# chongkuiqi/S2ANet

Hardware: AMD Instinct MI355X
Metric: 1024x1024 DOTA chips/sec (R-50-FPN S2ANet inference) (higher is better)
Workload: dtype f16; 1 GPU; BASELINE configs[2]: full R-50-FPN S2ANet inference, batch 8 of 1024x1024 synthetic uint8 chips per GPU; 3 independent batches in flight on 3 HIP streams; global_batch=8, num_classes=15, weights=seeded random init of the reference architecture; odm_cls bias calibrated, nms_candidate_cap=160000, nms_candidates_dropped=0, distinct_input_batches=3, fam_cls_branch=True, hip_graph=False, batches_in_flight=3, parallelism=dp1 (one process per GPU)

## Files before the change

### include/s2anet_hip.h

```cpp
#ifndef S2ANET_HIP_H_
#define S2ANET_HIP_H_

#include <stddef.h>
#include <stdint.h>

#ifdef __cplusplus
extern "C" {
#endif

#define S2A_OK 0
#define S2A_EINVAL (-1)
#define S2A_EWORKSPACE (-2)
#define S2A_EHIP (-3)
#define S2A_ENOTIMPL (-4)

#define S2A_DTYPE_F32 0
#define S2A_DTYPE_F16 1
#define S2A_DTYPE_F64 2

#define S2A_LAYOUT_NCHW 0
#define S2A_LAYOUT_NHWC 1

typedef void* s2a_stream_t;

// ... 258 lines not shown
int s2a_deform_conv_backward_typed(int dtype, const void* input, const void* offset, const void* grad_output,
                                   const void* weight, void* grad_input, void* grad_offset, float* grad_weight_f32,
                                   float scale, int64_t batch, int64_t channels, int64_t height, int64_t width,
                                   int64_t out_channels, void* workspace, size_t workspace_bytes, s2a_stream_t stream);

int s2a_conv3x3_tail1x1_f16(const void* x, const void* weight_frag, const void* bias, const void* tail_weight_frag,
                            const void* tail_bias, const void* residual, void* out, const void* chain_weight_frag,
                            const void* chain_bias, void* chain_out, int64_t chain_channels, int64_t batch, int64_t channels,
                            int64_t mid_channels, int64_t out_channels, int64_t height, int64_t width,
                            s2a_stream_t stream);

int s2a_conv1x1_chain_f16(const void* x, const void* weight_frag, const void* bias, const void* residual, void* out,
                          const void* chain_weight_frag, const void* chain_bias, void* chain_out, int64_t chain_channels,
                          int64_t batch, int64_t channels, int64_t out_channels, int64_t height, int64_t width,
                          s2a_stream_t stream);

int s2a_conv1x1_add_up2_f16(const void* x, const void* weight_frag, const void* bias, const void* coarse,
                            void* out, int64_t batch, int64_t channels, int64_t height, int64_t width,
                            int64_t out_channels, s2a_stream_t stream);
int s2a_sum_pool2x2_f16(const void* g, void* out, int64_t batch, int64_t height, int64_t width, int64_t channels,
                        s2a_stream_t stream);

int64_t s2a_pyramid_pixels(const s2a_pyramid* pyr, int64_t batch);
int s2a_conv3x3_pyramid_f16(const void* x, const void* weight_frag, const void* bias, const void* residual,
                            void* out, int64_t batch, int64_t channels, int64_t out_channels, int relu,
                            const s2a_pyramid* pyr, s2a_stream_t stream);
int s2a_conv3x3_head_pyramid_f16(const void* x, const void* weight_frag, const void* bias, void* out,
                                 const void* head_weight_frag, const void* head_bias, void* head_out,
                                 int64_t batch, int64_t channels, int64_t out_channels, int relu,
                                 const s2a_pyramid* pyr, s2a_stream_t stream);
// ... 125 lines not shown
```

### s2anet_amd/_lib.py

```python
import ctypes
import os
import subprocess

import torch

_HERE = os.path.dirname(os.path.abspath(__file__))
LIB_PATH = os.environ.get("S2A_LIB_PATH") or os.path.join(_HERE, "libs2anet_hip.so")

OK, EINVAL, EWORKSPACE, EHIP, ENOTIMPL = 0, -1, -2, -3, -4
DTYPE_F32, DTYPE_F16, DTYPE_F64 = 0, 1, 2
LAYOUT_NCHW, LAYOUT_NHWC = 0, 1

c_i64, c_int, c_f32, c_sz, c_vp = (ctypes.c_int64, ctypes.c_int, ctypes.c_float, ctypes.c_size_t,
                                   ctypes.c_void_p)


class DcnParams(ctypes.Structure):
    _fields_ = [("batch", c_i64), ("channels", c_i64), ("height", c_i64), ("width", c_i64),
                ("out_channels", c_i64),
                ("kW", c_int), ("kH", c_int), ("dW", c_int), ("dH", c_int), ("padW", c_int),
                ("padH", c_int), ("dilationW", c_int), ("dilationH", c_int), ("group", c_int),
                ("deformable_group", c_int), ("dtype", c_int), ("offset_dtype", c_int),
                ("layout", c_int), ("relu", c_int)]

# ... 137 lines not shown
                                               c_i64, c_vp, c_sz, c_vp]),
    "s2a_deform_conv_backward_input_f32_workspace_bytes": (c_sz, [c_i64, c_i64, c_i64, c_i64, c_i64]),
    "s2a_deform_conv_backward_weight_f32_workspace_bytes": (c_sz, [c_i64, c_i64, c_i64, c_i64, c_i64]),
    "s2a_deform_conv_backward_weight_f32": (c_int, [c_vp, c_vp, c_vp, c_vp, c_f32, c_i64, c_i64, c_i64, c_i64, c_i64,
                                                    c_vp, c_sz, c_vp]),
    "s2a_deform_conv_backward_input_f32": (c_int, [c_vp, c_vp, c_vp, c_vp, c_vp, c_vp, c_i64, c_i64, c_i64, c_i64, c_i64,
                                                   c_vp, c_sz, c_vp]),
    "s2a_deform_conv_backward_weight_f16": (c_int, [c_vp, c_vp, c_vp, c_vp, c_i64, c_i64, c_i64, c_i64, c_i64, c_vp, c_sz, c_vp]),
    "s2a_deform_conv_backward_input_f16": (c_int, [c_vp, c_vp, c_vp, c_vp, c_vp, c_vp, c_i64, c_i64, c_i64, c_i64, c_i64,
                                           c_vp, c_sz, c_vp]),
    "s2a_deformable_im2col": (c_int, [c_vp, c_vp, c_vp, ctypes.POINTER(DcnParams), c_vp]),
    "s2a_deformable_col2im": (c_int, [c_vp, c_vp, c_vp, ctypes.POINTER(DcnParams), c_vp]),
    "s2a_deformable_col2im_coord": (c_int, [c_vp, c_vp, c_vp, c_vp, ctypes.POINTER(DcnParams), c_vp]),
    "s2a_conv3x3_tail1x1_f16": (c_int, [c_vp] * 10 + [c_i64] * 7 + [c_vp]),
    "s2a_conv1x1_chain_f16": (c_int, [c_vp] * 8 + [c_i64] * 6 + [c_vp]),
    "s2a_conv1x1_add_up2_f16": (c_int, [c_vp, c_vp, c_vp, c_vp, c_vp, c_i64, c_i64, c_i64, c_i64, c_i64, c_vp]),
    "s2a_sum_pool2x2_f16": (c_int, [c_vp, c_vp, c_i64, c_i64, c_i64, c_i64, c_vp]),
    "s2a_pyramid_pixels": (c_i64, [ctypes.POINTER(Pyramid), c_i64]),
    "s2a_conv3x3_pyramid_f16": (c_int, [c_vp, c_vp, c_vp, c_vp, c_vp, c_i64, c_i64, c_i64, c_int,
                                        ctypes.POINTER(Pyramid), c_vp]),
    "s2a_conv3x3_head_pyramid_f16": (c_int, [c_vp, c_vp, c_vp, c_vp, c_vp, c_vp, c_vp, c_i64, c_i64, c_i64, c_int,
                                             ctypes.POINTER(Pyramid), c_vp]),
    "s2a_conv3x3_narrow_pyramid_f16": (c_int, [c_vp, c_vp, c_vp, c_vp, c_i64, c_i64, c_i64, c_int, ctypes.POINTER(Pyramid), c_vp]),
    "s2a_orconv_pool_pyramid_f16": (c_int, [c_vp, c_vp, c_vp, c_vp, c_vp, c_i64, c_i64, c_i64, ctypes.POINTER(Pyramid), c_vp]),
    "s2a_conv_wino_packed_elems": (c_i64, [c_i64, c_i64]),
    "s2a_conv_wino_pack_weight_f16": (c_int, [c_vp, c_i64, c_i64, c_vp, c_vp]),
    "s2a_conv3x3_wino_pyramid_f16": (c_int, [c_vp, c_vp, c_vp, c_vp, c_vp, c_i64, c_i64, c_i64, c_int,
                                             ctypes.POINTER(Pyramid), c_vp]),
    "s2a_quantize_e4m3": (c_int, [c_vp, c_vp, c_i64, c_i64, c_f32, c_vp]),
    "s2a_conv_pack_weight_fp8": (c_int, [c_vp, c_i64, c_i64, c_vp, c_vp]),
# ... 130 lines not shown
```

### s2anet_amd/csrc/conv_ops.hip

```cpp
#include <hip/hip_fp16.h>
#include <hip/hip_runtime.h>

#include <algorithm>
#include <cstdlib>
#include <type_traits>

#include "common.hpp"
#include "mfma_common.hpp"

namespace s2a {
namespace {

__global__ void k_pack_weight_frag(const _Float16* __restrict__ w, int O, int C, _Float16* __restrict__ wp,
                                   int taps = 9) {
  int64_t e = (int64_t)blockIdx.x * blockDim.x + threadIdx.x;
  int64_t total = (int64_t)O * C * taps;
  if (e >= total) return;
  const int G = O / 64;
  int j = (int)(e & 7);
  int lane = (int)((e >> 3) & 63);
  int kk = (int)((e >> 9) & 3);
  int mt = (int)((e >> 11) & 1);
  int64_t r = e >> 12;
  int g = (int)(r % G);
// ... 10 lines not shown
  _Float16* pool_out;
  const _Float16* head_w;
  const _Float16* head_b;
  _Float16* head_out;
  int store_main;
  const _Float16* tail_w;
  const _Float16* tail_b;
  const _Float16* tail_res;
  _Float16* tail_out;
  const _Float16* chain_w;
  const _Float16* chain_b;
  _Float16* chain_out;
  int chain_O;
};

template <int TAPS, int OG, int PH = 1, int SD = 1, bool TAIL = false, int HT = 0>
struct ConvCfg {
  static constexpr int kTH = (SD == 2 || HT) ? 4 : 8 * PH;
  static constexpr int kPos = (SD == 2 || HT) ? 64 : 128 * PH;
  static constexpr int kWaves = 4 * PH;
  static constexpr int kPW = SD == 2 ? 33 : kCPW;
  static constexpr int kNT = (kPos / 32) * OG / 4 / PH;
  static constexpr int kPix = TAPS == 9 ? ((kTH - 1) * SD + 3) * kPW : kPos;
  static constexpr int kDma = (kPix * 9 + 63) / 64;
  static constexpr int kPatchBytes = kDma * 1024;
  static constexpr int kOutRowB = OG * 128 + 16;
  static constexpr bool kWLds = PH == 2 && TAPS == 9;
  static constexpr int kWBuf = OG * 8192;
  static constexpr int kLoop0 = 2 * kPatchBytes + (kWLds ? 2 * kWBuf : 0);
  static constexpr int kLoop = (kWLds && OG == 1 && kPatchBytes + 9 * 8192 > kLoop0) ? kPatchBytes + 9 * 8192 : kLoop0;
  static constexpr int kLds0 = (kLoop > kPos * kOutRowB) ? kLoop : kPos * kOutRowB;
  static constexpr int kTailRowB = 528;
  static constexpr int kLds = (TAIL && kPos * kTailRowB > kLds0) ? kPos * kTailRowB : kLds0;
  static constexpr int kBiasBytes = TAIL ? 1024 : 512;
  static constexpr int kJ = (kDma + kWaves - 1) / kWaves;
};

template <int TAPS, int OG, int PH = 1, int SD = 1, bool TAIL = false, int HT = 0>
__global__ __launch_bounds__(256 * PH, PH == 1 ? 2 : 1) void k_conv_f16(const _Float16* __restrict__ x_,
                                                     const _Float16* __restrict__ wfrag,
                                                     const _Float16* __restrict__ bias,
                                                     const _Float16* __restrict__ residual_,
                                                     _Float16* __restrict__ out_, int64_t Ntot_, int C,
                                                     int H_, int W_, int Ho_, int Wo_, int cstride, int O,
                                                     int relu, unsigned x_bytes_, LevelTab lt, int res_up,
                                                     ConvExtra ex) {
  _Float16* pool_out_ = ex.pool_out;
  using T = _Float16;
  using V = f16x8;
  using Cfg = ConvCfg<TAPS, OG, PH, SD, TAIL, HT>;
  constexpr int NT = Cfg::kNT;
  static_assert(NT >= 1, "unsupported tile / group combination");
  static_assert(!HT || (TAPS == 9 && PH == 1 && SD == 1 && !TAIL), "half tiles: plain 3x3 / stride 1");
  static_assert(!TAIL || (TAPS == 9 && OG == 1 && SD == 1), "the fused 1x1 tail follows a 64-map 3x3/s1");
  constexpr int WPG = 4 / OG;
  constexpr int kThreads_ = 256 * PH;
  extern __shared__ __attribute__((aligned(16))) char smem[];
  const int tid = threadIdx.x, lane = tid & 63, wave = tid >> 6;
  const int wave4 = wave & 3, blk = wave >> 2;
  int64_t tile = xcd_remap(blockIdx.x, gridDim.x);
  const T* x = x_;
  const T* residual = residual_;
  T* out = out_;
  int64_t Ntot = Ntot_;
  int H = H_, W = W_, Ho = Ho_, Wo = Wo_;
  unsigned x_bytes = x_bytes_;
  if (TAPS == 9 && lt.n > 1) {
// ... 45 lines not shown
    }
    pvoff[j] = in ? (unsigned)(pix * row_bytes + q * 16) : 0x80000000u;
  }
  T* s_bias = reinterpret_cast<T*>(smem + Cfg::kLds);
  T bias_v = (T)0.f;
  if (bias && tid < Oloc) bias_v = bias[o0 + tid];
  T tail_bias_v = (T)0.f;
  V wt[2][4];
  if constexpr (TAIL) {
    if (tid < 256) tail_bias_v = ex.tail_b[tid];
    const V* tp = reinterpret_cast<const V*>(ex.tail_w) + (int64_t)wave4 * 8 * 64 + ((lane >> 4) & 1) * 128 + (lane >> 5) * 32 + (lane & 15);
#pragma unroll
    for (int f = 0; f < 8; f++) wt[f >> 2][f & 3] = tp[((f >> 2) * 4 + (f & 1)) * 64 + ((f >> 1) & 1) * 16];
  }
  auto patch_issue = [&](int cc) {
    char* P = smem + (cc & 1) * Cfg::kPatchBytes;
#pragma unroll
    for (int j = 0; j < Cfg::kJ; j++) {
      const int i = wave_u + Cfg::kWaves * j;
      if (i < Cfg::kDma)
        __builtin_amdgcn_raw_ptr_buffer_load_lds(rx, (__attribute__((address_space(3))) void*)(P + i * 1024), 16,
                                                 (int)pvoff[j], cc * 128, 0, 0);
    }
  };

  const int grp = wave4 / WPG, sub = wave4 % WPG;
  const bool wave_active = grp * 64 < Oloc;
  const int g = min(o0 / 64 + grp, G - 1);
  const V* wf_base = reinterpret_cast<const V*>(wfrag) + lane;
  V wA[2][4], wB[2][4];
  constexpr bool M16 = (TAPS == 9 && SD == 1) || (TAPS == 1 && OG == 4);
// ... 166 lines not shown
        if (t == 0 && cc + 1 < CC) patch_issue(cc + 1);
        compute_wl(Pc, t, wb + (s & 1) * Cfg::kWBuf);
        __syncthreads();
      }
    }
    }
  } else {
  patch_issue(0);
  load_w(0, wA);
  if (tid < 64 * OG) s_bias[tid] = bias_v;
  if constexpr (TAIL) { if (tid < 256) s_bias[64 + tid] = tail_bias_v; }
  __syncthreads();
  if constexpr (TAPS == 9) {
    for (int cc = 0; cc < CC; cc++) {
      const int s0 = cc * 9;
      const char* Pc = smem + (cc & 1) * Cfg::kPatchBytes;
#define S2A_TAP(T_, WCUR, WNEXT)                                                     \
      load_w(min(s0 + (T_) + 1, last), WNEXT);                                          \
      compute(Pc, (T_), WCUR);                                                          \
      __builtin_amdgcn_sched_barrier(0);
      S2A_TAP(0, wA, wB)
      S2A_TAP(1, wB, wA)
      S2A_TAP(2, wA, wB)
      S2A_TAP(3, wB, wA)
      S2A_TAP(4, wA, wB)
      S2A_TAP(5, wB, wA)
      if (cc + 1 < CC) patch_issue(cc + 1);
      S2A_TAP(6, wA, wB)
      S2A_TAP(7, wB, wA)
      S2A_TAP(8, wA, wB)
#undef S2A_TAP
      __syncthreads();
#pragma unroll
      for (int a = 0; a < 2; a++)
#pragma unroll
        for (int kk = 0; kk < 4; kk++) wA[a][kk] = wB[a][kk];
    }
  } else {
#define S2A_STAGE(C_, WCUR, WNEXT)                                                   \
    if ((C_) + 1 < CC) patch_issue((C_) + 1);                                           \
    load_w(min((C_) + 1, last), WNEXT);                                                 \
    compute(smem + ((C_) & 1) * Cfg::kPatchBytes, 0, WCUR);                             \
    __syncthreads();
    int cc = 0;
    for (; cc + 1 < CC; cc += 2) {
      S2A_STAGE(cc, wA, wB)
      S2A_STAGE(cc + 1, wB, wA)
// ... 666 lines not shown
    }
    stage_sync(issued);
#pragma unroll
    for (int i = 0; i < 4; i++) {
      const int idx = tid + 256 * i, pos = idx >> 3, col = idx & 7;
      const int y = cur.ty0 + (pos >> 4), xq = cur.tx0 + (pos & 15);
      V v;
#pragma unroll
      for (int e = 0; e < 8; e++) v[e] = (_Float16)0.f;
      if (col < 2) v = *reinterpret_cast<const V*>(so + pos * 32 + col * 16);
      if (y < cur.H && xq < cur.W) *reinterpret_cast<V*>(out + (cur.base + (int64_t)y * cur.W + xq) * 64 + col * 8) = v;
    }
  }
}

}
}

using namespace s2a;

namespace s2a {
namespace {
template <int TAPS, int OG, int PH = 1, int SD = 1, bool TAIL = false, int HT = 0>
int launch_conv(const _Float16* x, const _Float16* wfrag, const _Float16* bias, const _Float16* residual,
                _Float16* out, int64_t B, int C, int H, int W, int Ho, int Wo, int cstride, int O, int relu,
                hipStream_t st, const LevelTab* levels = nullptr, int64_t level_tiles = 0, int res_up = 0,
                ConvExtra ex = ConvExtra{nullptr, nullptr, nullptr, nullptr, 1}) {
  using Cfg = ConvCfg<TAPS, OG, PH, SD, TAIL, HT>;
  const int64_t Ntot = B * (int64_t)Ho * Wo;
  int64_t tiles = TAPS == 9 ? B * ((Wo + 15) / 16) * ((Ho + Cfg::kTH - 1) / Cfg::kTH) : (Ntot + Cfg::kPos - 1) / Cfg::kPos;
  LevelTab lt = {};
  if (levels) { lt = *levels; tiles = level_tiles; }
  dim3 grid((unsigned)tiles, (unsigned)((O + 64 * OG - 1) / (64 * OG)));
  auto kern = k_conv_f16<TAPS, OG, PH, SD, TAIL, HT>;
  S2A_HIP(hipFuncSetAttribute(reinterpret_cast<const void*>(kern), hipFuncAttributeMaxDynamicSharedMemorySize, Cfg::kLds + Cfg::kBiasBytes));
  kern<<<grid, 256 * PH, Cfg::kLds + Cfg::kBiasBytes, st>>>(x, wfrag, bias, residual, out, Ntot, C, H, W, Ho, Wo, cstride, O, relu,
                                     (unsigned)((uint64_t)B * H * W * C * 2), lt, res_up, ex);
  S2A_LAUNCH_CHECK();
  return S2A_OK;
}

struct ConvForm {
  int taps, og, ph, sd, tail, ht;
  bool operator==(const ConvForm& o) const {
    return taps == o.taps && og == o.og && ph == o.ph && sd == o.sd && tail == o.tail && ht == o.ht;
  }
};

struct ConvCall {
  const _Float16 *x, *wfrag, *bias, *residual;
  _Float16* out;
  int64_t B;
  int C, H, W, Ho, Wo, cstride, O, relu;
  hipStream_t st;
  const LevelTab* levels = nullptr;
  int64_t level_tiles = 0;
  int res_up = 0;
  ConvExtra ex = ConvExtra{nullptr, nullptr, nullptr, nullptr, 1};
  template <int TAPS, int OG, int PH = 1, int SD = 1, bool TAIL = false, int HT = 0>
  int run() const {
    return launch_conv<TAPS, OG, PH, SD, TAIL, HT>(x, wfrag, bias, residual, out, B, C, H, W, Ho, Wo, cstride, O, relu, st, levels,
                                                   level_tiles, res_up, ex);
  }
  int run(const ConvForm& f) const {
#define S2A_CONV_FORM(TAPS, OG, PH, SD, TAIL, HT) \
  if (f == ConvForm{TAPS, OG, PH, SD, TAIL, HT}) return run<TAPS, OG, PH, SD, TAIL, HT>()
    S2A_CONV_FORM(9, 4, 1, 2, 0, 0);
    S2A_CONV_FORM(9, 2, 1, 2, 0, 0);
    S2A_CONV_FORM(9, 2, 2, 1, 0, 0);
    S2A_CONV_FORM(9, 1, 2, 1, 0, 0);
    S2A_CONV_FORM(9, 4, 2, 1, 0, 0);
    S2A_CONV_FORM(9, 4, 1, 1, 0, 1);
    S2A_CONV_FORM(9, 2, 1, 1, 0, 1);
    S2A_CONV_FORM(9, 4, 1, 1, 0, 0);
    S2A_CONV_FORM(9, 2, 1, 1, 0, 0);
    S2A_CONV_FORM(9, 1, 1, 1, 0, 0);
    S2A_CONV_FORM(1, 4, 1, 2, 0, 0);
    S2A_CONV_FORM(1, 4, 1, 1, 0, 0);
    S2A_CONV_FORM(1, 2, 1, 1, 0, 0);
    S2A_CONV_FORM(1, 1, 1, 1, 0, 0);
    S2A_CONV_FORM(9, 1, 2, 1, 1, 0);
    S2A_CONV_FORM(9, 1, 1, 1, 1, 0);
#undef S2A_CONV_FORM
    s2a::set_error("conv: no kernel of form <%d, %d, %d, %d, %d, %d>", f.taps, f.og, f.ph, f.sd, f.tail, f.ht);
    return S2A_EINVAL;
  }
};

inline int env_ph(const char* name, int ph) {
  const char* f = getenv(name);
  return f ? (atoi(f) == 2 ? 2 : 1) : ph;
}
inline bool env_flag(const char* name, bool on) {
  const char* f = getenv(name);
  return f ? atoi(f) != 0 : on;
}
inline int conv_og(int64_t out_channels) { return out_channels % 256 == 0 ? 4 : (out_channels % 128 == 0 ? 2 : 1); }

ConvForm conv_form_nhwc(int64_t batch, int64_t channels, int64_t height, int64_t width, int64_t out_channels, int ksize,
                        int stride) {
  const int64_t Ho = (height - 1) / stride + 1, Wo = (width - 1) / stride + 1;
  const int og = conv_og(out_channels);
  const int64_t groups = (out_channels + 64 * og - 1) / (64 * og);
  if (ksize == 3 && stride == 2) return {9, og == 4 ? 4 : 2, 1, 2, 0, 0};
  if (ksize == 3 && og < 4 && channels % 64 == 0) {
    const int64_t tiles16 = batch * ((Wo + 15) / 16) * ((Ho + 15) / 16) * groups;
    if (env_ph("S2A_CONV_PH_NARROW", tiles16 >= 256 ? 2 : 1) == 2) return {9, og, 2, 1, 0, 0};
  }
  if (ksize == 3 && og == 4 && channels % 64 == 0) {
    const int64_t tiles16 = batch * ((Wo + 15) / 16) * ((Ho + 15) / 16) * groups;
    if (env_ph("S2A_CONV_PH", tiles16 >= 512 ? 2 : 1) == 2) return {9, 4, 2, 1, 0, 0};
  }
  if (ksize == 3 && og >= 2) {
    const int64_t wgs128 = batch * ((Wo + 15) / 16) * ((Ho + 7) / 8) * groups;
    if (env_flag("S2A_CONV3_HALF", wgs128 < 256)) return {9, og, 1, 1, 0, 1};
  }
  if (ksize == 3) return {9, og, 1, 1, 0, 0};
  if (og == 4) {
    const int64_t wgs128 = (batch * Ho * Wo + 127) / 128 * groups;
// ... 130 lines not shown
  if (batch == 0) return S2A_OK;
  S2A_CHECK_ARG(x && weight_frag && bias && out && chain_weight_frag, "conv1x1_chain: NULL tensor");
  S2A_CHECK_ARG(((uintptr_t)x % 16) == 0 && ((uintptr_t)out % 16) == 0 && ((uintptr_t)weight_frag % 16) == 0 &&
                ((uintptr_t)bias % 8) == 0 && ((uintptr_t)residual % 16) == 0 && ((uintptr_t)chain_weight_frag % 16) == 0 &&
                ((uintptr_t)chain_bias % 8) == 0 && ((uintptr_t)chain_out % 16) == 0,
                "conv1x1_chain: tensors must be 16-byte aligned");
  const int64_t P = batch * height * width;
  const _Float16 *X = (const _Float16*)x, *Wf = (const _Float16*)weight_frag, *Bi = (const _Float16*)bias,
                 *R = (const _Float16*)residual, *Cw = (const _Float16*)chain_weight_frag, *Cb = (const _Float16*)chain_bias;
  hipStream_t st = as_stream(stream);
  if (channels == 256) return launch_conv1x1_chain<4, 256>(X, Wf, Bi, R, (_Float16*)out, Cw, Cb, (_Float16*)chain_out, P, st);
  if (chain_channels == 128) return launch_conv1x1_chain<2, 128>(X, Wf, Bi, R, (_Float16*)out, Cw, Cb, (_Float16*)chain_out, P, st);
  return launch_conv1x1_chain<2, 256>(X, Wf, Bi, R, (_Float16*)out, Cw, Cb, (_Float16*)chain_out, P, st);
}

extern "C" int s2a_conv1x1_add_up2_f16(const void* x, const void* weight_frag, const void* bias, const void* coarse,
                                       void* out, int64_t batch, int64_t channels, int64_t height, int64_t width,
                                       int64_t out_channels, s2a_stream_t stream) {
  S2A_CHECK_ARG(batch >= 0 && channels > 0 && out_channels > 0 && height > 0 && width > 0, "conv_add_up2: bad shape");
  S2A_CHECK_ARG(height % 2 == 0 && width % 2 == 0, "conv_add_up2: the map must be exactly twice the coarse map");
  S2A_CHECK_ARG(channels % 64 == 0 && out_channels % 64 == 0, "conv_add_up2: channel counts must be multiples of 64");
  const uint64_t x_bytes = (uint64_t)batch * height * width * channels * 2;
  S2A_CHECK_ARG(x_bytes < (1ull << 31) && (uint64_t)batch * height * width * out_channels * 2 < (1ull << 31),
                "conv_add_up2: tensor too large for 32-bit offsets");
  if (batch == 0) return S2A_OK;
  S2A_CHECK_ARG(x && weight_frag && coarse && out, "conv_add_up2: NULL tensor");
  S2A_CHECK_ARG(((uintptr_t)x % 16) == 0 && ((uintptr_t)out % 16) == 0 && ((uintptr_t)weight_frag % 16) == 0 &&
                ((uintptr_t)bias % 2) == 0 && ((uintptr_t)coarse % 16) == 0, "conv_add_up2: tensors must be 16-byte aligned");
  const ConvCall c{(const _Float16*)x, (const _Float16*)weight_frag, (const _Float16*)bias, (const _Float16*)coarse,
                   (_Float16*)out, batch, (int)channels, (int)height, (int)width, (int)height, (int)width, 1, (int)out_channels, 0,
// ... 109 lines not shown
```

### s2anet_amd/detector.py

```python
import math
import os

import torch
import torch.nn as nn
import torch.nn.functional as F

from .fused import Conv3Chain, FusedConv2d, bottleneck_chain_ok, bottleneck_tail, bottleneck_tail_ok, conv3_chain_ok
from .head import S2ANetHead


class BottleNeck(nn.Module):
    expansion = 4

    def __init__(self, inplanes, planes, stride=1, downsample=None):
        super().__init__()
        self.conv1 = nn.Conv2d(inplanes, planes, kernel_size=1, stride=1, bias=False)
        self.bn1 = nn.BatchNorm2d(planes)
        self.conv2 = nn.Conv2d(planes, planes, kernel_size=3, stride=stride, padding=1, bias=False)
        self.bn2 = nn.BatchNorm2d(planes)
        self.conv3 = nn.Conv2d(planes, planes * self.expansion, kernel_size=1, bias=False)
        self.bn3 = nn.BatchNorm2d(planes * self.expansion)
        self.relu = nn.ReLU(inplace=True)
        self.downsample = downsample
        self.stride = stride

    def forward(self, x):
        return self.forward_chain(x)[0]

    def forward_chain(self, x, pre=None, nxt=None):
        residual = x
        if isinstance(self.conv3, FusedConv2d):
            out = pre if pre is not None else self.conv1(x)
            if self.downsample is not None:
                residual = self.downsample(x)
            if bottleneck_tail_ok(out, self.conv2, self.conv3, residual):
                if isinstance(nxt, BottleNeck) and bottleneck_chain_ok(nxt.conv1):
                    return bottleneck_tail(out, self.conv2, self.conv3, residual, nxt.conv1)
                return bottleneck_tail(out, self.conv2, self.conv3, residual), None
            if isinstance(nxt, BottleNeck) and conv3_chain_ok(self.conv3, nxt.conv1):
                ch = Conv3Chain(nxt.conv1)
                return self.conv3(self.conv2(out), residual, chain=ch), ch.out
            return self.conv3(self.conv2(out), residual), None
        return self._forward_plain(x), None

    def _forward_plain(self, x):
        residual = x
        out = self.relu(self.bn1(self.conv1(x)))
        out = self.relu(self.bn2(self.conv2(out)))
        out = self.bn3(self.conv3(out))
# ... 293 lines not shown
```

### s2anet_amd/fused.py

```python
import torch
import torch.nn as nn
import torch.nn.functional as F

from . import _lib


def _needs_grad(*tensors):
    return torch.is_grad_enabled() and any(t is not None and t.requires_grad for t in tensors)


def bias_act_(y, bias, residual=None, relu=False, out=None):
    _lib.require_cuda(y, bias, residual)
    B, C, H, W = y.shape
    if out is not None:
        assert out.shape == y.shape and out.dtype == y.dtype and out.permute(0, 2, 3, 1).is_contiguous()
    grad = _needs_grad(y, bias, residual)
    if grad and out is not None:
        raise RuntimeError("bias_act_(out=...) writes a caller's buffer and has no backward: call it under torch.no_grad()")
    ok = (not grad and y.is_contiguous(memory_format=torch.channels_last) and
          C % (8 if y.dtype == torch.float16 else 4) == 0 and y.dtype in (torch.float16, torch.float32) and
          (residual is None or (residual.shape == y.shape and residual.dtype == y.dtype and
                                residual.is_contiguous(memory_format=torch.channels_last))))
    if not ok:
        y = y + bias.view(1, -1, 1, 1).to(y.dtype)
# ... 72 lines not shown
    return out


def conv_wino_f16(x, packed_wino, bias, out_channels, relu=False, pool=False):
    from .pyramid import PyramidLayout, conv3x3_wino
    B, C, H, W = x.shape
    assert x.dtype == torch.float16 and x.is_contiguous(memory_format=torch.channels_last)
    lay = PyramidLayout(B, [(H, W)], [1.0])
    b = None if bias is None else bias.to(torch.float16).contiguous()
    r = conv3x3_wino(lay, x.permute(0, 2, 3, 1).reshape(-1, C), packed_wino, b, out_channels, relu, pool)
    if pool:
        return (r[0].view(B, H, W, out_channels).permute(0, 3, 1, 2), r[1].view(B, H, W, out_channels // 8).permute(0, 3, 1, 2))
    return r.view(B, H, W, out_channels).permute(0, 3, 1, 2)


def conv_f16(x, packed_weight, bias, out_channels, ksize, stride=1, relu=False, residual=None, out=None, chain=None):
    B, C, H, W = x.shape
    Ho, Wo = (H - 1) // stride + 1, (W - 1) // stride + 1
    O_real = out_channels
    if out_channels < 64:
        assert residual is None
        out_channels = 64
    if out is None:
        out = torch.empty((B, out_channels, Ho, Wo), dtype=torch.float16, device=x.device,
                          memory_format=torch.channels_last)
    else:
        assert out.shape == (B, out_channels, Ho, Wo) and out.dtype == torch.float16 and \
            out.permute(0, 2, 3, 1).is_contiguous()
    b = None if bias is None else bias.to(torch.float16).contiguous()
    if b is not None and b.numel() < out_channels:
        b = torch.cat([b, b.new_zeros(out_channels - b.numel())])
    if residual is not None:
        assert residual.shape == out.shape and residual.dtype == torch.float16 and \
            residual.is_contiguous(memory_format=torch.channels_last)
    if chain is not None and ksize == 1 and stride == 1 and relu and b is not None and \
            (C, out_channels, chain.conv.out_channels) in CONV3_CHAIN_SHAPES and out.numel() * 2 < (1 << 31):
        wc, bc, _ = chain.conv.packed_args()
        chain.out = torch.empty((B, chain.conv.out_channels, H, W), dtype=torch.float16, device=x.device,
                                memory_format=torch.channels_last)
        with torch.cuda.device(x.device):
            _lib.check(_lib.lib().s2a_conv1x1_chain_f16(_lib.ptr(x), _lib.ptr(packed_weight), _lib.ptr(b), _lib.ptr(residual),
                                                        _lib.ptr(out), _lib.ptr(wc), _lib.ptr(bc), _lib.ptr(chain.out),
                                                        chain.conv.out_channels, B, C, out_channels, H, W,
                                                        _lib.stream_ptr(x.device)))
        return out
    with torch.cuda.device(x.device):
        _lib.check(_lib.lib().s2a_conv_nhwc_f16(_lib.ptr(x), _lib.ptr(packed_weight), _lib.ptr(b), _lib.ptr(residual),
                                                _lib.ptr(out), B, C, H, W, out_channels, int(ksize), int(stride),
                                                int(bool(relu)), _lib.stream_ptr(x.device)))
    return out if O_real == out_channels else out[:, :O_real]


CONV3_CHAIN_SHAPES = {(128, 512, 128), (128, 512, 256), (256, 1024, 256)}


class Conv3Chain:

    def __init__(self, conv):
        self.conv, self.out = conv, None


def conv3_chain_ok(conv3, conv1):
    import os
    def plain(c):
        return (isinstance(c, FusedConv2d) and tuple(c.kernel_size) == (1, 1) and tuple(c.stride) == (1, 1) and
                tuple(c.padding) == (0, 0) and tuple(c.dilation) == (1, 1) and c.groups == 1 and c.bias is not None and
                c.fuse_relu and c.weight.dtype == torch.float16)
    return (not torch.is_grad_enabled() and not os.environ.get("S2A_NO_CONV3_CHAIN") and plain(conv3) and plain(conv1) and
            conv1.in_channels == conv3.out_channels and
            (conv3.in_channels, conv3.out_channels, conv1.out_channels) in CONV3_CHAIN_SHAPES)


def bottleneck_tail_ok(x, conv2, conv3, residual):
    import os
    return (not torch.is_grad_enabled() and not os.environ.get("S2A_NO_FUSED_TAIL") and
            isinstance(conv2, FusedConv2d) and isinstance(conv3, FusedConv2d) and
            conv2.in_channels == 64 and conv2.out_channels == 64 and conv3.out_channels == 256 and
            conv2.fuse_relu and conv3.fuse_relu and conv2.bias is not None and conv3.bias is not None and
            own_conv_ok(x, 64, 64, conv2.kernel_size, conv2.stride, conv2.padding, conv2.dilation, conv2.groups) and
            tuple(conv2.kernel_size) == (3, 3) and tuple(conv2.stride) == (1, 1) and
            tuple(conv3.kernel_size) == (1, 1) and tuple(conv3.stride) == (1, 1) and
            x.shape[0] * x.shape[2] * x.shape[3] * 512 < (1 << 31) and
            (residual is None or (residual.dtype == torch.float16 and residual.shape[1] == 256 and
                                  residual.shape[2:] == x.shape[2:] and
                                  residual.is_contiguous(memory_format=torch.channels_last))))
# ... 359 lines not shown
        if not hasattr(self, "_packed"):
            self._packed = PackedWeightCache()
        w, sc = self._packed.get_fp8(self.weight, in_scale)
        return w, sc, self._packed.get_bias_f32(self.bias), self.out_channels

    def wino_ok(self):
        return (tuple(self.kernel_size) == (3, 3) and tuple(self.stride) == (1, 1) and tuple(self.padding) == (1, 1) and
                tuple(self.dilation) == (1, 1) and self.groups == 1 and self.out_channels % 64 == 0 and
                self.in_channels % 32 == 0)

    def packed_args_wino(self):
        if not hasattr(self, "_packed"):
            self._packed = PackedWeightCache()
        return self._packed.get_wino(self.weight), self._packed.get_bias(self.bias, self.out_channels), self.out_channels

    def forward(self, x, residual=None, out=None, chain=None):
        if out is None and self.own_grad and _needs_grad(x, self.weight, self.bias, residual) and \
                train_conv_ok(x, self, residual):
            return FusedConvFunction.apply(x, self.weight, self.bias, residual, self.fuse_relu)
        if out is None and self.own_grad_strided and _needs_grad(x, self.weight, self.bias, residual) and \
                train_conv_strided_ok(x, self, residual):
            return FusedConvS2Function.apply(x, self.weight, self.bias, residual, self.fuse_relu)
        if out is None and residual is None and self.own_grad and _lib.deterministic() and _needs_grad(x, self.weight, self.bias):
            pad = train_pad_widths(x, self)
            if pad is not None:
                return padded_train_conv(x, self.weight, self.bias, self.fuse_relu, *pad)
        if out is not None:
            assert x.is_cuda and self.bias is not None and not torch.is_grad_enabled() and not own_conv_ok(
                x, self.in_channels, self.out_channels, self.kernel_size, self.stride, self.padding, self.dilation, self.groups)
            y = F.conv2d(x, self.weight, None, self.stride, self.padding, self.dilation, self.groups)
            return bias_act_(y, self.bias, residual, self.fuse_relu, out=out)
        if not torch.is_grad_enabled() and own_conv_ok(
                x, self.in_channels, self.out_channels, self.kernel_size, self.stride, self.padding,
                self.dilation, self.groups) and (residual is None or (
                    residual.dtype == torch.float16 and residual.is_contiguous(memory_format=torch.channels_last))):
            if not hasattr(self, "_packed"):
                self._packed = PackedWeightCache()
            kw = {} if chain is None else {"chain": chain}
            return conv_f16(x, self._packed.get(self.weight), self._packed.get_bias(self.bias, max(64, self.out_channels)),
                            self.out_channels, self.kernel_size[0], self.stride[0], self.fuse_relu, residual, **kw)
        if (not x.is_cuda) or self.bias is None:
            y = super().forward(x)
            if residual is not None:
                y = y + residual
            return F.relu(y) if self.fuse_relu else y
        y = F.conv2d(x, self.weight, None, self.stride, self.padding, self.dilation, self.groups)
        return bias_act_(y, self.bias, residual, self.fuse_relu)


def stem_pack_weight(weight):
    w = weight.detach().to(torch.float16).contiguous()
    assert tuple(w.shape) == (64, 3, 7, 7)
    L = _lib.lib()
# ... 74 lines not shown
```

Before: 1958 chips/s.

## Fuse layer1 conv1 and downsample 1x1 convs; single-buffer stride-2 3x3 patches

Adds a kernel that reads the 64-channel input tile once and computes both the bottleneck conv1 (64->64, ReLU) and the downsample projection (64->256) in one launch, writing both outputs. This removes a second full read of the input and one kernel launch in the first layer1 block. Separately, the stride-2 3x3 conv gets a single-patch-buffer variant that is chosen when the grid is large, cutting LDS use to raise occupancy. The cost is serialized patch loads, since prefetch overlap within a workgroup is lost.

```diff
diff --git a/include/s2anet_hip.h b/include/s2anet_hip.h
--- a/include/s2anet_hip.h
+++ b/include/s2anet_hip.h
@@ -296,6 +296,11 @@
                           const void* chain_weight_frag, const void* chain_bias, void* chain_out, int64_t chain_channels,
                           int64_t batch, int64_t channels, int64_t out_channels, int64_t height, int64_t width,
                           s2a_stream_t stream);
+
+int s2a_conv1x1_pair_f16(const void* x, const void* weight_a_frag, const void* bias_a, void* out_a,
+                         const void* weight_b_frag, const void* bias_b, void* out_b, int64_t batch, int64_t channels,
+                         int64_t height, int64_t width, int64_t out_a_channels, int64_t out_b_channels,
+                         s2a_stream_t stream);
 
 int s2a_conv1x1_add_up2_f16(const void* x, const void* weight_frag, const void* bias, const void* coarse,
                             void* out, int64_t batch, int64_t channels, int64_t height, int64_t width,
diff --git a/s2anet_amd/_lib.py b/s2anet_amd/_lib.py
--- a/s2anet_amd/_lib.py
+++ b/s2anet_amd/_lib.py
@@ -175,6 +175,7 @@
     "s2a_deformable_col2im_coord": (c_int, [c_vp, c_vp, c_vp, c_vp, ctypes.POINTER(DcnParams), c_vp]),
     "s2a_conv3x3_tail1x1_f16": (c_int, [c_vp] * 10 + [c_i64] * 7 + [c_vp]),
     "s2a_conv1x1_chain_f16": (c_int, [c_vp] * 8 + [c_i64] * 6 + [c_vp]),
+    "s2a_conv1x1_pair_f16": (c_int, [c_vp] * 7 + [c_i64] * 6 + [c_vp]),
     "s2a_conv1x1_add_up2_f16": (c_int, [c_vp, c_vp, c_vp, c_vp, c_vp, c_i64, c_i64, c_i64, c_i64, c_i64, c_vp]),
     "s2a_sum_pool2x2_f16": (c_int, [c_vp, c_vp, c_i64, c_i64, c_i64, c_i64, c_vp]),
     "s2a_pyramid_pixels": (c_i64, [ctypes.POINTER(Pyramid), c_i64]),
diff --git a/s2anet_amd/csrc/conv_ops.hip b/s2anet_amd/csrc/conv_ops.hip
--- a/s2anet_amd/csrc/conv_ops.hip
+++ b/s2anet_amd/csrc/conv_ops.hip
@@ -48,7 +48,7 @@
   int chain_O;
 };
 
-template <int TAPS, int OG, int PH = 1, int SD = 1, bool TAIL = false, int HT = 0>
+template <int TAPS, int OG, int PH = 1, int SD = 1, bool TAIL = false, int HT = 0, int NB = 2>
 struct ConvCfg {
   static constexpr int kTH = (SD == 2 || HT) ? 4 : 8 * PH;
   static constexpr int kPos = (SD == 2 || HT) ? 64 : 128 * PH;
@@ -61,7 +61,7 @@
   static constexpr int kOutRowB = OG * 128 + 16;
   static constexpr bool kWLds = PH == 2 && TAPS == 9;
   static constexpr int kWBuf = OG * 8192;
-  static constexpr int kLoop0 = 2 * kPatchBytes + (kWLds ? 2 * kWBuf : 0);
+  static constexpr int kLoop0 = NB * kPatchBytes + (kWLds ? 2 * kWBuf : 0);
   static constexpr int kLoop = (kWLds && OG == 1 && kPatchBytes + 9 * 8192 > kLoop0) ? kPatchBytes + 9 * 8192 : kLoop0;
   static constexpr int kLds0 = (kLoop > kPos * kOutRowB) ? kLoop : kPos * kOutRowB;
   static constexpr int kTailRowB = 528;
@@ -70,7 +70,7 @@
   static constexpr int kJ = (kDma + kWaves - 1) / kWaves;
 };
 
-template <int TAPS, int OG, int PH = 1, int SD = 1, bool TAIL = false, int HT = 0>
+template <int TAPS, int OG, int PH = 1, int SD = 1, bool TAIL = false, int HT = 0, int NB = 2>
 __global__ __launch_bounds__(256 * PH, PH == 1 ? 2 : 1) void k_conv_f16(const _Float16* __restrict__ x_,
                                                      const _Float16* __restrict__ wfrag,
                                                      const _Float16* __restrict__ bias,
@@ -82,9 +82,10 @@
   _Float16* pool_out_ = ex.pool_out;
   using T = _Float16;
   using V = f16x8;
-  using Cfg = ConvCfg<TAPS, OG, PH, SD, TAIL, HT>;
+  using Cfg = ConvCfg<TAPS, OG, PH, SD, TAIL, HT, NB>;
   constexpr int NT = Cfg::kNT;
   static_assert(NT >= 1, "unsupported tile / group combination");
+  static_assert(NB == 2 || (NB == 1 && TAPS == 9 && SD == 2), "one patch buffer: the stride-2 3x3 only");
   static_assert(!HT || (TAPS == 9 && PH == 1 && SD == 1 && !TAIL), "half tiles: plain 3x3 / stride 1");
   static_assert(!TAIL || (TAPS == 9 && OG == 1 && SD == 1), "the fused 1x1 tail follows a 64-map 3x3/s1");
   constexpr int WPG = 4 / OG;
@@ -160,7 +161,7 @@
     for (int f = 0; f < 8; f++) wt[f >> 2][f & 3] = tp[((f >> 2) * 4 + (f & 1)) * 64 + ((f >> 1) & 1) * 16];
   }
   auto patch_issue = [&](int cc) {
-    char* P = smem + (cc & 1) * Cfg::kPatchBytes;
+    char* P = smem + (cc & (NB - 1)) * Cfg::kPatchBytes;
 #pragma unroll
     for (int j = 0; j < Cfg::kJ; j++) {
       const int i = wave_u + Cfg::kWaves * j;
@@ -357,7 +358,7 @@
   if constexpr (TAPS == 9) {
     for (int cc = 0; cc < CC; cc++) {
       const int s0 = cc * 9;
-      const char* Pc = smem + (cc & 1) * Cfg::kPatchBytes;
+      const char* Pc = smem + (cc & (NB - 1)) * Cfg::kPatchBytes;
 #define S2A_TAP(T_, WCUR, WNEXT)                                                     \
       load_w(min(s0 + (T_) + 1, last), WNEXT);                                          \
       compute(Pc, (T_), WCUR);                                                          \
@@ -368,12 +369,19 @@
       S2A_TAP(3, wB, wA)
       S2A_TAP(4, wA, wB)
       S2A_TAP(5, wB, wA)
-      if (cc + 1 < CC) patch_issue(cc + 1);
+      if (NB == 2 && cc + 1 < CC) patch_issue(cc + 1);
       S2A_TAP(6, wA, wB)
       S2A_TAP(7, wB, wA)
       S2A_TAP(8, wA, wB)
 #undef S2A_TAP
       __syncthreads();
+      if constexpr (NB == 1) {
+        if (cc + 1 < CC) {
+          patch_issue(cc + 1);
+          asm volatile("s_waitcnt vmcnt(0)" ::: "memory");
+          __syncthreads();
+        }
+      }
 #pragma unroll
       for (int a = 0; a < 2; a++)
 #pragma unroll
@@ -1070,6 +1078,142 @@
   }
 }
 
+
+constexpr int kPairTile = 128 * kRowBytes;
+constexpr int kPairRowB = 528;
+constexpr int kPairLds = 128 * kPairRowB;
+static_assert(kPairTile == 18 * 1024 && kPairTile <= kPairLds, "pair: tile inside the staging area");
+__global__ __launch_bounds__(256, 2) void k_conv1x1_pair_f16(const _Float16* __restrict__ x,
+                                                             const _Float16* __restrict__ wa_frag,
+                                                             const _Float16* __restrict__ bias_a,
+                                                             _Float16* __restrict__ out_a,
+                                                             const _Float16* __restrict__ wb_frag,
+                                                             const _Float16* __restrict__ bias_b,
+                                                             _Float16* __restrict__ out_b, int64_t Ntot,
+                                                             unsigned x_bytes) {
+  using T = _Float16;
+  using V = f16x8;
+  using h2e = __attribute__((ext_vector_type(2))) _Float16;
+  using h4e = __attribute__((ext_vector_type(4))) _Float16;
+  extern __shared__ __attribute__((aligned(16))) char smem[];
+  const int tid = threadIdx.x, lane = tid & 63;
+  const int wave = __builtin_amdgcn_readfirstlane(tid >> 6);
+  const int64_t g0 = (int64_t)xcd_remap(blockIdx.x, gridDim.x) * 128;
+  T* s_bias = reinterpret_cast<T*>(smem + kPairLds);
+  const __amdgpu_buffer_rsrc_t rx = __builtin_amdgcn_make_buffer_rsrc(const_cast<T*>(x), 0, (int)x_bytes, 0x00020000);
+#pragma unroll
+  for (int j = 0; j < 5; j++) {
+    const int i = wave + 4 * j;
+    const int v = i * 64 + lane, p = v / 9, q = v % 9;
+    const bool in = q < 8 && g0 + p < Ntot;
+    const unsigned off = in ? (unsigned)((g0 + p) * 128 + q * 16) : 0x80000000u;
+    if (i < 18)
+      __builtin_amdgcn_raw_ptr_buffer_load_lds(rx, (__attribute__((address_space(3))) void*)(smem + i * 1024), 16, (int)off, 0, 0, 0);
+  }
+  const T ba = tid < 64 ? bias_a[tid] : (T)0.f, bb = bias_b[tid];
+  V wa[2][4], wb[2][4];
+  {
+    const V* p = reinterpret_cast<const V*>(wa_frag) + lane;
+#pragma unroll
+    for (int a = 0; a < 2; a++)
+#pragma unroll
+      for (int kk = 0; kk < 4; kk++) wa[a][kk] = p[(a * 4 + kk) * 64];
+    const V* pb = reinterpret_cast<const V*>(wb_frag) + wave * 8 * 64 + ((lane >> 4) & 1) * 128 + (lane >> 5) * 32 + (lane & 15);
+#pragma unroll
+    for (int f = 0; f < 8; f++) wb[f >> 2][f & 3] = pb[((f >> 2) * 4 + (f & 1)) * 64 + ((f >> 1) & 1) * 16];
+  }
+  if (tid < 64) s_bias[tid] = ba;
+  s_bias[64 + tid] = bb;
+  asm volatile("s_waitcnt vmcnt(0)" ::: "memory");
+  __syncthreads();
+
+  const int posA = 32 * wave + (lane & 31);
+  h4e ha[2][4];
+  {
+    f32x16 acc[2];
+#pragma unroll
+    for (int a = 0; a < 2; a++)
+#pragma unroll
+      for (int r = 0; r < 16; r++) acc[a][r] = 0.f;
+    const char* fb = smem + posA * kRowBytes + (lane >> 5) * 16;
+#pragma unroll
+    for (int kk = 0; kk < 4; kk++) {
+      const V pf = *reinterpret_cast<const V*>(fb + kk * 32);
+#pragma unroll
+      for (int a = 0; a < 2; a++) acc[a] = __builtin_amdgcn_mfma_f32_32x32x16_f16(wa[a][kk], pf, acc[a], 0, 0, 0);
+    }
+#pragma unroll
+    for (int a = 0; a < 2; a++)
+#pragma unroll
+      for (int rq = 0; rq < 4; rq++) {
+        const h4e bq = *reinterpret_cast<const h4e*>(s_bias + 32 * a + 8 * rq + 4 * (lane >> 5));
+        h2e lo = {(_Float16)(acc[a][rq * 4] + (float)bq[0]), (_Float16)(acc[a][rq * 4 + 1] + (float)bq[1])};
+        h2e hi = {(_Float16)(acc[a][rq * 4 + 2] + (float)bq[2]), (_Float16)(acc[a][rq * 4 + 3] + (float)bq[3])};
+        lo = __builtin_elementwise_max(lo, h2e{(_Float16)0.f, (_Float16)0.f});
+        hi = __builtin_elementwise_max(hi, h2e{(_Float16)0.f, (_Float16)0.f});
+        ha[a][rq] = h4e{lo[0], lo[1], hi[0], hi[1]};
+      }
+  }
+  const int kg16 = lane >> 4, i16 = lane & 15;
+  const int pix16 = (i16 >= 4 && i16 < 12) ? (((i16 - 4) >> 1) * 4 + (i16 & 1))
+                                           : (((i16 & 3) >> 1) * 4 + 2 + (i16 & 1) + (i16 >= 12 ? 8 : 0));
+  f32x4 acc16[4][8];
+#pragma unroll
+  for (int a = 0; a < 4; a++)
+#pragma unroll
+    for (int b = 0; b < 8; b++)
+#pragma unroll
+      for (int r = 0; r < 4; r++) acc16[a][b][r] = 0.f;
+  {
+    const char* fb = smem + pix16 * kRowBytes + (kg16 & 1) * 64 + (kg16 >> 1) * 16;
+#pragma unroll
+    for (int ks = 0; ks < 2; ks++)
+#pragma unroll
+      for (int bh = 0; bh < 8; bh += 4) {
+        V pf[4];
+#pragma unroll
+        for (int b = 0; b < 4; b++) pf[b] = *reinterpret_cast<const V*>(fb + (bh + b) * 16 * kRowBytes + ks * 32);
+#pragma unroll
+        for (int a = 0; a < 4; a++)
+#pragma unroll
+          for (int b = 0; b < 4; b++)
+            acc16[a][bh + b] = __builtin_amdgcn_mfma_f32_16x16x32_f16(wb[(a * 2 + ks) >> 2][(a * 2 + ks) & 3], pf[b], acc16[a][bh + b], 0, 0, 0);
+      }
+  }
+  __syncthreads();
+#pragma unroll
+  for (int a = 0; a < 2; a++)
+#pragma unroll
+    for (int rq = 0; rq < 4; rq++)
+      *reinterpret_cast<h4e*>(smem + posA * kRowBytes + (32 * a + 8 * rq + 4 * (lane >> 5)) * 2) = ha[a][rq];
+  __syncthreads();
+#pragma unroll
+  for (int i = 0; i < 4; i++) {
+    const int idx = tid + 256 * i, pos = idx >> 3, col = idx & 7;
+    if (g0 + pos < Ntot)
+      *reinterpret_cast<V*>(out_a + (g0 + pos) * 64 + col * 8) = *reinterpret_cast<const V*>(smem + pos * kRowBytes + col * 16);
+  }
+  __syncthreads();
+#pragma unroll
+  for (int a = 0; a < 4; a++) {
+    const int och = wave * 64 + 16 * a + 4 * kg16;
+    const h4e bq = *reinterpret_cast<const h4e*>(s_bias + 64 + och);
+#pragma unroll
+    for (int b = 0; b < 8; b++) {
+      const h2e lo = {(_Float16)(acc16[a][b][0] + (float)bq[0]), (_Float16)(acc16[a][b][1] + (float)bq[1])};
+      const h2e hi = {(_Float16)(acc16[a][b][2] + (float)bq[2]), (_Float16)(acc16[a][b][3] + (float)bq[3])};
+      *reinterpret_cast<h4e*>(smem + (16 * b + pix16) * kPairRowB + och * 2) = h4e{lo[0], lo[1], hi[0], hi[1]};
+    }
+  }
+  __syncthreads();
+#pragma unroll
+  for (int i = 0; i < 16; i++) {
+    const int idx = tid + 256 * i, pos = idx >> 5, col = idx & 31;
+    if (g0 + pos < Ntot)
+      *reinterpret_cast<V*>(out_b + (g0 + pos) * 256 + col * 8) = *reinterpret_cast<const V*>(smem + pos * kPairRowB + col * 16);
+  }
+}
+
 }
 }
 
@@ -1077,18 +1221,18 @@
 
 namespace s2a {
 namespace {
-template <int TAPS, int OG, int PH = 1, int SD = 1, bool TAIL = false, int HT = 0>
+template <int TAPS, int OG, int PH = 1, int SD = 1, bool TAIL = false, int HT = 0, int NB = 2>
 int launch_conv(const _Float16* x, const _Float16* wfrag, const _Float16* bias, const _Float16* residual,
                 _Float16* out, int64_t B, int C, int H, int W, int Ho, int Wo, int cstride, int O, int relu,
                 hipStream_t st, const LevelTab* levels = nullptr, int64_t level_tiles = 0, int res_up = 0,
                 ConvExtra ex = ConvExtra{nullptr, nullptr, nullptr, nullptr, 1}) {
-  using Cfg = ConvCfg<TAPS, OG, PH, SD, TAIL, HT>;
+  using Cfg = ConvCfg<TAPS, OG, PH, SD, TAIL, HT, NB>;
   const int64_t Ntot = B * (int64_t)Ho * Wo;
   int64_t tiles = TAPS == 9 ? B * ((Wo + 15) / 16) * ((Ho + Cfg::kTH - 1) / Cfg::kTH) : (Ntot + Cfg::kPos - 1) / Cfg::kPos;
   LevelTab lt = {};
   if (levels) { lt = *levels; tiles = level_tiles; }
   dim3 grid((unsigned)tiles, (unsigned)((O + 64 * OG - 1) / (64 * OG)));
-  auto kern = k_conv_f16<TAPS, OG, PH, SD, TAIL, HT>;
+  auto kern = k_conv_f16<TAPS, OG, PH, SD, TAIL, HT, NB>;
   S2A_HIP(hipFuncSetAttribute(reinterpret_cast<const void*>(kern), hipFuncAttributeMaxDynamicSharedMemorySize, Cfg::kLds + Cfg::kBiasBytes));
   kern<<<grid, 256 * PH, Cfg::kLds + Cfg::kBiasBytes, st>>>(x, wfrag, bias, residual, out, Ntot, C, H, W, Ho, Wo, cstride, O, relu,
                                      (unsigned)((uint64_t)B * H * W * C * 2), lt, res_up, ex);
@@ -1098,8 +1242,9 @@
 
 struct ConvForm {
   int taps, og, ph, sd, tail, ht;
+  int bufs = 2;
   bool operator==(const ConvForm& o) const {
-    return taps == o.taps && og == o.og && ph == o.ph && sd == o.sd && tail == o.tail && ht == o.ht;
+    return taps == o.taps && og == o.og && ph == o.ph && sd == o.sd && tail == o.tail && ht == o.ht && bufs == o.bufs;
   }
 };
 
@@ -1113,9 +1258,9 @@
   int64_t level_tiles = 0;
   int res_up = 0;
   ConvExtra ex = ConvExtra{nullptr, nullptr, nullptr, nullptr, 1};
-  template <int TAPS, int OG, int PH = 1, int SD = 1, bool TAIL = false, int HT = 0>
+  template <int TAPS, int OG, int PH = 1, int SD = 1, bool TAIL = false, int HT = 0, int NB = 2>
   int run() const {
-    return launch_conv<TAPS, OG, PH, SD, TAIL, HT>(x, wfrag, bias, residual, out, B, C, H, W, Ho, Wo, cstride, O, relu, st, levels,
+    return launch_conv<TAPS, OG, PH, SD, TAIL, HT, NB>(x, wfrag, bias, residual, out, B, C, H, W, Ho, Wo, cstride, O, relu, st, levels,
                                                    level_tiles, res_up, ex);
   }
   int run(const ConvForm& f) const {
@@ -1123,6 +1268,8 @@
   if (f == ConvForm{TAPS, OG, PH, SD, TAIL, HT}) return run<TAPS, OG, PH, SD, TAIL, HT>()
     S2A_CONV_FORM(9, 4, 1, 2, 0, 0);
     S2A_CONV_FORM(9, 2, 1, 2, 0, 0);
+    if (f == ConvForm{9, 4, 1, 2, 0, 0, 1}) return run<9, 4, 1, 2, false, 0, 1>();
+    if (f == ConvForm{9, 2, 1, 2, 0, 0, 1}) return run<9, 2, 1, 2, false, 0, 1>();
     S2A_CONV_FORM(9, 2, 2, 1, 0, 0);
     S2A_CONV_FORM(9, 1, 2, 1, 0, 0);
     S2A_CONV_FORM(9, 4, 2, 1, 0, 0);
@@ -1138,7 +1285,8 @@
     S2A_CONV_FORM(9, 1, 2, 1, 1, 0);
     S2A_CONV_FORM(9, 1, 1, 1, 1, 0);
 #undef S2A_CONV_FORM
-    s2a::set_error("conv: no kernel of form <%d, %d, %d, %d, %d, %d>", f.taps, f.og, f.ph, f.sd, f.tail, f.ht);
+    s2a::set_error("conv: no kernel of form <%d, %d, %d, %d, %d, %d>, %d patch buffers", f.taps, f.og, f.ph, f.sd, f.tail, f.ht,
+                   f.bufs);
     return S2A_EINVAL;
   }
 };
@@ -1158,7 +1306,13 @@
   const int64_t Ho = (height - 1) / stride + 1, Wo = (width - 1) / stride + 1;
   const int og = conv_og(out_channels);
   const int64_t groups = (out_channels + 64 * og - 1) / (64 * og);
-  if (ksize == 3 && stride == 2) return {9, og == 4 ? 4 : 2, 1, 2, 0, 0};
+  if (ksize == 3 && stride == 2) {
+    const int og2 = og == 4 ? 4 : 2;
+    const int64_t wgs = batch * ((Wo + 15) / 16) * ((Ho + 3) / 4) * ((out_channels + 64 * og2 - 1) / (64 * og2));
+    int bufs = wgs > 256 ? 1 : 2;
+    if (const char* f = getenv("S2A_CONV_S2_BUFS")) bufs = atoi(f) == 1 ? 1 : 2;
+    return {9, og2, 1, 2, 0, 0, bufs};
+  }
   if (ksize == 3 && og < 4 && channels % 64 == 0) {
     const int64_t tiles16 = batch * ((Wo + 15) / 16) * ((Ho + 15) / 16) * groups;
     if (env_ph("S2A_CONV_PH_NARROW", tiles16 >= 256 ? 2 : 1) == 2) return {9, og, 2, 1, 0, 0};
@@ -1319,6 +1473,31 @@
   return launch_conv1x1_chain<2, 256>(X, Wf, Bi, R, (_Float16*)out, Cw, Cb, (_Float16*)chain_out, P, st);
 }
 
+extern "C" int s2a_conv1x1_pair_f16(const void* x, const void* weight_a_frag, const void* bias_a, void* out_a,
+                                    const void* weight_b_frag, const void* bias_b, void* out_b, int64_t batch,
+                                    int64_t channels, int64_t height, int64_t width, int64_t out_a_channels,
+                                    int64_t out_b_channels, s2a_stream_t stream) {
+  S2A_CHECK_ARG(batch >= 0 && height > 0 && width > 0, "conv1x1_pair: bad shape");
+  S2A_CHECK_ARG(channels == 64 && out_a_channels == 64 && out_b_channels == 256,
+                "conv1x1_pair: built for (K, Oa, Ob) = (64, 64, 256)");
+  S2A_CHECK_ARG((uint64_t)batch * height * width * out_b_channels * 2 < (1ull << 31),
+                "conv1x1_pair: tensor too large for 32-bit offsets");
+  if (batch == 0) return S2A_OK;
+  S2A_CHECK_ARG(x && weight_a_frag && bias_a && out_a && weight_b_frag && bias_b && out_b, "conv1x1_pair: NULL tensor");
+  S2A_CHECK_ARG(((uintptr_t)x % 16) == 0 && ((uintptr_t)out_a % 16) == 0 && ((uintptr_t)out_b % 16) == 0 &&
+                ((uintptr_t)weight_a_frag % 16) == 0 && ((uintptr_t)weight_b_frag % 16) == 0 &&
+                ((uintptr_t)bias_a % 8) == 0 && ((uintptr_t)bias_b % 8) == 0,
+                "conv1x1_pair: tensors must be 16-byte aligned");
+  const int64_t P = batch * height * width;
+  const int lds = kPairLds + 640;
+  S2A_HIP(hipFuncSetAttribute(reinterpret_cast<const void*>(k_conv1x1_pair_f16), hipFuncAttributeMaxDynamicSharedMemorySize, lds));
+  k_conv1x1_pair_f16<<<dim3((unsigned)((P + 127) / 128)), 256, lds, as_stream(stream)>>>(
+      (const _Float16*)x, (const _Float16*)weight_a_frag, (const _Float16*)bias_a, (_Float16*)out_a,
+      (const _Float16*)weight_b_frag, (const _Float16*)bias_b, (_Float16*)out_b, P, (unsigned)((uint64_t)P * 64 * 2));
+  S2A_LAUNCH_CHECK();
+  return S2A_OK;
+}
+
 extern "C" int s2a_conv1x1_add_up2_f16(const void* x, const void* weight_frag, const void* bias, const void* coarse,
                                        void* out, int64_t batch, int64_t channels, int64_t height, int64_t width,
                                        int64_t out_channels, s2a_stream_t stream) {
diff --git a/s2anet_amd/detector.py b/s2anet_amd/detector.py
--- a/s2anet_amd/detector.py
+++ b/s2anet_amd/detector.py
@@ -5,7 +5,8 @@
 import torch.nn as nn
 import torch.nn.functional as F
 
-from .fused import Conv3Chain, FusedConv2d, bottleneck_chain_ok, bottleneck_tail, bottleneck_tail_ok, conv3_chain_ok
+from .fused import (Conv3Chain, ConvPair, FusedConv2d, bottleneck_chain_ok, bottleneck_tail, bottleneck_tail_ok,
+                    conv3_chain_ok, conv_pair_ok)
 from .head import S2ANetHead
 
 
@@ -30,9 +31,15 @@
     def forward_chain(self, x, pre=None, nxt=None):
         residual = x
         if isinstance(self.conv3, FusedConv2d):
-            out = pre if pre is not None else self.conv1(x)
+            pr = None
+            if pre is None and isinstance(self.downsample, nn.Sequential) and len(self.downsample) == 1 and \
+                    conv_pair_ok(self.conv1, self.downsample[0]):
+                pr = ConvPair(self.downsample[0])
+                out = self.conv1(x, pair=pr)
+            else:
+                out = pre if pre is not None else self.conv1(x)
             if self.downsample is not None:
-                residual = self.downsample(x)
+                residual = pr.out if pr is not None and pr.out is not None else self.downsample(x)
             if bottleneck_tail_ok(out, self.conv2, self.conv3, residual):
                 if isinstance(nxt, BottleNeck) and bottleneck_chain_ok(nxt.conv1):
                     return bottleneck_tail(out, self.conv2, self.conv3, residual, nxt.conv1)
diff --git a/s2anet_amd/fused.py b/s2anet_amd/fused.py
--- a/s2anet_amd/fused.py
+++ b/s2anet_amd/fused.py
@@ -110,7 +110,8 @@
     return r.view(B, H, W, out_channels).permute(0, 3, 1, 2)
 
 
-def conv_f16(x, packed_weight, bias, out_channels, ksize, stride=1, relu=False, residual=None, out=None, chain=None):
+def conv_f16(x, packed_weight, bias, out_channels, ksize, stride=1, relu=False, residual=None, out=None, chain=None,
+             pair=None):
     B, C, H, W = x.shape
     Ho, Wo = (H - 1) // stride + 1, (W - 1) // stride + 1
     O_real = out_channels
@@ -140,6 +141,18 @@
                                                         chain.conv.out_channels, B, C, out_channels, H, W,
                                                         _lib.stream_ptr(x.device)))
         return out
+    if pair is not None and chain is None and out_channels == O_real and not torch.is_grad_enabled() and \
+            tuple(pair.conv.kernel_size) == (1, 1) and tuple(pair.conv.stride) == (1, 1) and \
+            conv_pair_shapes_ok(C, out_channels, pair.conv.out_channels, ksize, stride, relu, b is not None,
+                                residual is not None, B * H * W):
+        wp, bp, _ = pair.conv.packed_args()
+        pair.out = torch.empty((B, pair.conv.out_channels, H, W), dtype=torch.float16, device=x.device,
+                               memory_format=torch.channels_last)
+        with torch.cuda.device(x.device):
+            _lib.check(_lib.lib().s2a_conv1x1_pair_f16(_lib.ptr(x), _lib.ptr(packed_weight), _lib.ptr(b), _lib.ptr(out),
+                                                       _lib.ptr(wp), _lib.ptr(bp), _lib.ptr(pair.out), B, C, H, W,
+                                                       out_channels, pair.conv.out_channels, _lib.stream_ptr(x.device)))
+        return out
     with torch.cuda.device(x.device):
         _lib.check(_lib.lib().s2a_conv_nhwc_f16(_lib.ptr(x), _lib.ptr(packed_weight), _lib.ptr(b), _lib.ptr(residual),
                                                 _lib.ptr(out), B, C, H, W, out_channels, int(ksize), int(stride),
@@ -165,6 +178,28 @@
     return (not torch.is_grad_enabled() and not os.environ.get("S2A_NO_CONV3_CHAIN") and plain(conv3) and plain(conv1) and
             conv1.in_channels == conv3.out_channels and
             (conv3.in_channels, conv3.out_channels, conv1.out_channels) in CONV3_CHAIN_SHAPES)
+
+
+class ConvPair:
+
+    def __init__(self, conv):
+        self.conv, self.out = conv, None
+
+
+def conv_pair_shapes_ok(C, O, O2, ksize, stride, relu, has_bias, has_residual, positions):
+    return ((C, O, O2) == (64, 64, 256) and ksize == 1 and stride == 1 and bool(relu) and bool(has_bias) and
+            not has_residual and 0 <= positions * 512 < (1 << 31))
+
+
+def conv_pair_ok(conv1, down):
+    import os
+    def plain(c, relu):
+        return (isinstance(c, FusedConv2d) and tuple(c.kernel_size) == (1, 1) and tuple(c.stride) == (1, 1) and
+                tuple(c.padding) == (0, 0) and tuple(c.dilation) == (1, 1) and c.groups == 1 and c.bias is not None and
+                bool(c.fuse_relu) == relu and c.weight.dtype == torch.float16)
+    return (not torch.is_grad_enabled() and not os.environ.get("S2A_NO_CONV_PAIR") and plain(conv1, True) and
+            plain(down, False) and (conv1.in_channels, conv1.out_channels) == (64, 64) and
+            (down.in_channels, down.out_channels) == (64, 256))
 
 
 def bottleneck_tail_ok(x, conv2, conv3, residual):
@@ -554,7 +589,7 @@
             self._packed = PackedWeightCache()
         return self._packed.get_wino(self.weight), self._packed.get_bias(self.bias, self.out_channels), self.out_channels
 
-    def forward(self, x, residual=None, out=None, chain=None):
+    def forward(self, x, residual=None, out=None, chain=None, pair=None):
         if out is None and self.own_grad and _needs_grad(x, self.weight, self.bias, residual) and \
                 train_conv_ok(x, self, residual):
             return FusedConvFunction.apply(x, self.weight, self.bias, residual, self.fuse_relu)
@@ -577,6 +612,8 @@
             if not hasattr(self, "_packed"):
                 self._packed = PackedWeightCache()
             kw = {} if chain is None else {"chain": chain}
+            if pair is not None:
+                kw["pair"] = pair
             return conv_f16(x, self._packed.get(self.weight), self._packed.get_bias(self.bias, max(64, self.out_channels)),
                             self.out_channels, self.kernel_size[0], self.stride[0], self.fuse_relu, residual, **kw)
         if (not x.is_cuda) or self.bias is None:
```

New measurement: 1972 chips/s, median of 6. No clear change (+0.7%).
